# codex-storage/nim-groth16

Measured on AMD Instinct MI355X. Metric: proofs/sec (BN254 Groth16, 2^20-constraint circuit), higher is better.
Workload: dtype u32 (254-bit Montgomery: 8x32-bit limbs; 9x29-bit limbs in the bucket accumulation); 1 GPU; BN254 2^20-constraint synthetic R1CS (squaring chain, m=2^20-2), full prove: buildABC + 6 NTT + 4 G1 MSM + 1 G2 MSM, snarkjs flavour, 1 proof/step/GPU (3 proofs in flight per GPU, one shared key); mode=replica, nvars=1048576, domain_log2=20

## Files before the change

### include/g16hip.h

```cpp
#ifndef G16HIP_H
#define G16HIP_H

#include <stddef.h>
#include <stdint.h>

#ifdef __cplusplus
extern "C" {
#endif

#define G16_OK 0
#define G16_EINVAL (-1)
#define G16_ENODEV (-2)
#define G16_EHIP (-3)
#define G16_ENOMEM (-4)
#define G16_ESELFTEST (-5)

typedef struct g16_ctx g16_ctx;
typedef struct g16_points g16_points;

#define G16_SCALARS_MONT 1u
#define G16_SCALARS_STD 0u
#define G16_SCALARS_DEVICE 2u
#define G16_OUT_PARTIAL 4u
#define G16_OUT_DEVICE 8u
// ... 98 lines not shown
  const void *pointsA1, *pointsB1;
  const void* pointsB2;
  const void* pointsC1;
  const void* pointsH1;
  const g16_coeff* coeffs;
  size_t ncoeffs;
  const void *alpha1, *beta1, *delta1;
  const void *beta2, *delta2;
  uint32_t shard_index, shard_count;
} g16_pkey_desc;
typedef struct {
  uint8_t pi_a[64];
  uint8_t pi_b[128];
  uint8_t pi_c[64];
} g16_proof;
int32_t g16_pkey_create(g16_ctx* ctx, const g16_pkey_desc* desc, g16_pkey** out);
int32_t g16_pkey_create_zkey(g16_ctx* ctx, const g16_pkey_desc* desc, const void* section4, size_t section4_bytes,
                             g16_pkey** out);
int32_t g16_pkey_create_lean(g16_ctx* ctx, const g16_pkey_desc* desc, uint32_t table_stride, g16_pkey** out);
int32_t g16_pkey_create_zkey_lean(g16_ctx* ctx, const g16_pkey_desc* desc, const void* section4, size_t section4_bytes,
                                  uint32_t table_stride, g16_pkey** out);
void g16_pkey_destroy(g16_pkey* key);
int32_t g16_pkey_inf_counts(const g16_pkey* key, size_t out[8]);
int32_t g16_prove(g16_ctx* ctx, const g16_pkey* key, const void* witness, uint32_t flags, const void* mask_r,
                  const void* mask_s, g16_proof* out);
#define G16_PARTIALS_BYTES 768
int32_t g16_prove_partials(g16_ctx* ctx, const g16_pkey* key, const void* witness, uint32_t flags, void* out_partials);
int32_t g16_prove_combine(g16_ctx* ctx, const g16_pkey* key, const void* partials, size_t count, uint32_t flags,
                          const void* mask_r, const void* mask_s, g16_proof* out);
int32_t g16_prove_partials_begin(g16_ctx* ctx, const g16_pkey* key, const void* witness, uint32_t flags,
                                 uint32_t task_mask, void* d_task_out);
int32_t g16_prove_partials_end(g16_ctx* ctx, const g16_pkey* key, const void* d_a1_slice, const void* d_b1_slice,
                               const void* d_c1_slice, uint32_t flags, void* out_partials);
int32_t g16_build_abc(g16_ctx* ctx, const g16_pkey* key, const void* witness, uint32_t flags, void* out_abc);
int32_t g16_pkey_abc_info(const g16_pkey* key, size_t out[11]);
int32_t g16_spmv_fr(g16_ctx* ctx, const uint32_t* row, const uint32_t* col, const void* val, size_t nnz, const void* x,
                    size_t ncols, size_t nrows, void* y);

typedef struct g16_group g16_group;
typedef struct g16_group_pkey g16_group_pkey;
int32_t g16_group_create(const int32_t* devices, int32_t ndev, g16_group** out);
void g16_group_destroy(g16_group* group);
int32_t g16_group_size(const g16_group* group);
const char* g16_group_last_error(const g16_group* group);
int32_t g16_group_pkey_create(g16_group* group, const g16_pkey_desc* desc, g16_group_pkey** out);
int32_t g16_group_pkey_create_lean(g16_group* group, const g16_pkey_desc* desc, uint32_t table_stride,
// ... 71 lines not shown
```

### nim_groth16_amd/_lib.py

```python
from __future__ import annotations

import ctypes
import json
import os
import weakref

_HERE = os.path.dirname(os.path.abspath(__file__))

G16_OK, G16_EINVAL, G16_ENODEV, G16_EHIP, G16_ENOMEM, G16_ESELFTEST, G16_EBUSY = 0, -1, -2, -3, -4, -5, -6
SCALARS_MONT, SCALARS_STD, SCALARS_DEVICE, OUT_PARTIAL, OUT_DEVICE, NO_HOST_SYNC = 1, 0, 2, 4, 8, 32
PARTIALS_BYTES = 768

SYMBOLS = [
    "g16_ctx_create", "g16_ctx_destroy", "g16_last_error", "g16_ctx_set_stream", "g16_ctx_synchronize",
    "g16_selftest", "g16_msm_g1", "g16_msm_g2", "g16_msm_g1_dev", "g16_msm_g2_dev",
    "g16_msm_g1_partial_dev", "g16_msm_g2_partial_dev", "g16_g1_sum_partials", "g16_g2_sum_partials",
    "g16_points_register_g1", "g16_points_register_g2", "g16_points_register_g1_dev",
    "g16_points_register_g2_dev", "g16_points_release", "g16_points_count", "g16_points_inf_count", "g16_points_info", "g16_msm_points",
    "g16_points_check_g1", "g16_points_check_g2", "g16_fixed_base_g1", "g16_fixed_base_g2", "g16_quotient", "g16_quotient_dev", "g16_pkey_create",
    "g16_pkey_create_zkey", "g16_pkey_destroy", "g16_pkey_inf_counts", "g16_prove", "g16_build_abc", "g16_pkey_abc_info", "g16_spmv_fr", "g16_prove_partials", "g16_prove_combine",
    "g16_prove_partials_begin", "g16_prove_partials_end",
    "g16_ntt_fr", "g16_ntt_fr_dev", "g16_profile_enable", "g16_profile_reset", "g16_profile_report", "g16_profile_clock",
    "g16_vkey_create", "g16_vkey_destroy", "g16_verify", "g16_verify_batch", "g16_pairing",
    "g16_ctx_cancel", "g16_group_create", "g16_group_destroy", "g16_group_size", "g16_group_last_error",
    "g16_group_pkey_create", "g16_group_pkey_destroy", "g16_group_prove",
    "g16_prover_create", "g16_prover_destroy", "g16_prover_last_error", "g16_prover_submit", "g16_prover_poll",
    "g16_prover_collect", "g16_host_alloc", "g16_host_free",
    "g16_points_register_g1_lean", "g16_points_register_g2_lean", "g16_points_register_g1_lean_dev",
    "g16_points_register_g2_lean_dev", "g16_points_table_bytes", "g16_points_plan", "g16_pkey_create_lean",
    "g16_pkey_create_zkey_lean", "g16_group_pkey_create_lean",
    "g16_setup_log2_domain", "g16_fake_setup", "g16_lagrange_fr", "g16_powers_fr",
    "g16_points_audit_g1", "g16_points_audit_g2", "g16_points_pairs_check", "g16_key_audit",
]
VERIFY_SUBGROUP = 16
GT_BYTES = 384


class PkeyDesc(ctypes.Structure):
    _fields_ = [("nvars", ctypes.c_uint32), ("npubs", ctypes.c_uint32), ("log2_domain", ctypes.c_uint32),
                ("flavour", ctypes.c_uint32),
                ("pointsA1", ctypes.c_void_p), ("pointsB1", ctypes.c_void_p), ("pointsB2", ctypes.c_void_p),
                ("pointsC1", ctypes.c_void_p), ("pointsH1", ctypes.c_void_p),
                ("coeffs", ctypes.c_void_p), ("ncoeffs", ctypes.c_size_t),
                ("alpha1", ctypes.c_void_p), ("beta1", ctypes.c_void_p), ("delta1", ctypes.c_void_p),
                ("beta2", ctypes.c_void_p), ("delta2", ctypes.c_void_p),
                ("shard_index", ctypes.c_uint32), ("shard_count", ctypes.c_uint32)]


class VkeyDesc(ctypes.Structure):
    _fields_ = [("npubs", ctypes.c_uint32), ("alpha1", ctypes.c_void_p), ("beta2", ctypes.c_void_p),
                ("gamma2", ctypes.c_void_p), ("delta2", ctypes.c_void_p), ("pointsIC", ctypes.c_void_p)]


class SetupDesc(ctypes.Structure):
    _fields_ = [("nvars", ctypes.c_uint32), ("npubs", ctypes.c_uint32), ("nconstraints", ctypes.c_uint32),
# ... 128 lines not shown
    for name in ("g16_msm_g1", "g16_msm_g2", "g16_msm_g1_dev", "g16_msm_g2_dev",
                 "g16_msm_g1_partial_dev", "g16_msm_g2_partial_dev"):
        getattr(lib, name).argtypes = [vp, vp, u32, vp, sz, vp]
    for name in ("g16_g1_sum_partials", "g16_g2_sum_partials"):
        getattr(lib, name).argtypes = [vp, vp, sz, vp]
    for name in ("g16_points_register_g1", "g16_points_register_g2", "g16_points_register_g1_dev",
                 "g16_points_register_g2_dev"):
        getattr(lib, name).argtypes = [vp, vp, sz, ctypes.POINTER(vp)]
    for name in ("g16_points_register_g1_lean", "g16_points_register_g2_lean", "g16_points_register_g1_lean_dev",
                 "g16_points_register_g2_lean_dev"):
        getattr(lib, name).argtypes = [vp, vp, sz, u32, ctypes.POINTER(vp)]
    lib.g16_points_table_bytes.argtypes = [vp, ctypes.POINTER(sz)]
    lib.g16_points_plan.argtypes = [ctypes.c_int, sz, u32, ctypes.POINTER(u32), ctypes.POINTER(u32), ctypes.POINTER(sz)]
    lib.g16_pkey_create_lean.argtypes = [vp, ctypes.POINTER(PkeyDesc), u32, ctypes.POINTER(vp)]
    lib.g16_pkey_create_zkey_lean.argtypes = [vp, ctypes.POINTER(PkeyDesc), vp, sz, u32, ctypes.POINTER(vp)]
    lib.g16_group_pkey_create_lean.argtypes = [vp, ctypes.POINTER(PkeyDesc), u32, ctypes.POINTER(vp)]
    lib.g16_points_release.argtypes = [vp]
    lib.g16_points_release.restype = None
    lib.g16_points_count.argtypes = [vp]
    lib.g16_points_count.restype = sz
    lib.g16_points_inf_count.argtypes = [vp]
    lib.g16_points_inf_count.restype = sz
    lib.g16_pkey_inf_counts.argtypes = [vp, ctypes.POINTER(sz)]
    lib.g16_points_info.argtypes = [vp, ctypes.POINTER(u32), ctypes.POINTER(u32)]
    lib.g16_msm_points.argtypes = [vp, vp, vp, u32, vp]
    lib.g16_points_check_g1.argtypes = [vp, vp, sz, ctypes.POINTER(sz)]
    lib.g16_points_check_g2.argtypes = [vp, vp, sz, ctypes.POINTER(sz)]
    lib.g16_fixed_base_g1.argtypes = [vp, vp, u32, sz, vp]
    lib.g16_fixed_base_g2.argtypes = [vp, vp, u32, sz, vp]
    lib.g16_quotient.argtypes = [vp, vp, vp, vp, u32, u32, vp]
    lib.g16_quotient_dev.argtypes = [vp, vp, vp, vp, u32, u32, vp]
    lib.g16_pkey_create.argtypes = [vp, ctypes.POINTER(PkeyDesc), ctypes.POINTER(vp)]
    lib.g16_pkey_create_zkey.argtypes = [vp, ctypes.POINTER(PkeyDesc), vp, sz, ctypes.POINTER(vp)]
    lib.g16_pkey_destroy.argtypes = [vp]
    lib.g16_pkey_destroy.restype = None
    lib.g16_prove.argtypes = [vp, vp, vp, u32, vp, vp, vp]
    lib.g16_build_abc.argtypes = [vp, vp, vp, u32, vp]
    lib.g16_pkey_abc_info.argtypes = [vp, ctypes.POINTER(sz)]
    lib.g16_spmv_fr.argtypes = [vp, vp, vp, vp, sz, vp, sz, sz, vp]
    lib.g16_prove_partials.argtypes = [vp, vp, vp, u32, vp]
    lib.g16_prove_combine.argtypes = [vp, vp, vp, sz, u32, vp, vp, vp]
    lib.g16_prove_partials_begin.argtypes = [vp, vp, vp, u32, u32, vp]
    lib.g16_prove_partials_end.argtypes = [vp, vp, vp, vp, vp, u32, vp]
    lib.g16_ntt_fr.argtypes = [vp, vp, vp, u32, i32]
    lib.g16_ntt_fr_dev.argtypes = [vp, vp, vp, u32, i32]
    lib.g16_vkey_create.argtypes = [vp, ctypes.POINTER(VkeyDesc), ctypes.POINTER(vp)]
# ... 360 lines not shown
        if out is not None:
            c._check(c._lib.g16_prove_partials_end(c._h, self._h, ptr(a1), ptr(b1), ptr(c1),
                                                   OUT_DEVICE | (NO_HOST_SYNC if nosync else 0), _buf(out)))
            return None
        buf = ctypes.create_string_buffer(PARTIALS_BYTES)
        c._check(c._lib.g16_prove_partials_end(c._h, self._h, ptr(a1), ptr(b1), ptr(c1), 0, buf))
        return buf.raw

    def prove_combine(self, partials, count: int, r: bytes = None, s: bytes = None, device: bool = False, ctx=None):
        c = ctx or self.ctx
        out = ctypes.create_string_buffer(256)
        c._check(c._lib.g16_prove_combine(c._h, self._h, _buf(partials), count, SCALARS_DEVICE if device else 0,
                                          _buf(r) if r else None, _buf(s) if s else None, out))
        raw = out.raw
        return raw[0:64], raw[64:192], raw[192:256]

    def inf_counts(self) -> dict:
        out = (ctypes.c_size_t * 8)()
        self.ctx._check(self.ctx._lib.g16_pkey_inf_counts(self._h, out))
        v = list(out)
        return {"A1": v[0], "B1": v[1], "B2": v[2], "C1": v[3], "H1": v[4], "B1_and_B2": v[5],
                "compact_A": bool(v[6]), "compact_B": bool(v[7])}

    def abc_info(self) -> dict:
        out = (ctypes.c_size_t * 11)()
        self.ctx._check(self.ctx._lib.g16_pkey_abc_info(self._h, out))
        v = list(out)
        names = ("L<=1", "L=2", "L<=4", "L<=8", "L<=16", "L<=32", "L<=64", "L<=128", "L>128")
        return {"ncoeffs": v[0], "dict_values": v[1], "rows_by_terms": dict(zip(names, v[2:]))}

    def build_abc(self, witness: bytes, mont: bool = True, ctx=None):
        c = ctx or self.ctx
        self._check_len(witness)
        n = 1 << self.log2n
        out = ctypes.create_string_buffer(3 * n * 32)
        c._check(c._lib.g16_build_abc(c._h, self._h, _buf(witness), SCALARS_MONT if mont else 0, out))
        raw = out.raw
        return raw[: 32 * n], raw[32 * n: 64 * n], raw[64 * n:]

    def _free(self):
        if self._h:
            self.ctx._lib.g16_pkey_destroy(self._h)
        self._h = None

    destroy = _free

# ... 271 lines not shown
```

### nim_groth16_amd/csrc/g16_env.hpp

```cpp
#pragma once

struct G16Env {
  int msm_window = 0;
  int table_window = 0;
  int msm_seg = 0;
  char msm_sort = 0;
  int g1_lanes[3] = {3, 2, 0};
  char stream_prio[7] = "lhllln";
  int red_slice_log2 = 0;
  int inf_compact_pct = 10;
  int r2_width = -1;
  int ntt_tile = 2048;
  int quotient_first = 1;
  int lanes_after_quotient = 0;
  int g1_batch = 0;
  int mtab = 2;
  int chain_ch = 1;
  int tail_quad = 1;
  int red_chunk = 0;
  int cu_split = 0;
  int heavy_grid = 0;
  int cz_on_the_fly = 1;
  int abc_dict = 1;
  int g2_first = -1;
};
```

### nim_groth16_amd/csrc/g16hip.hip

```cpp
#include "g16_internal.hpp"
#include "ec.cuh"

using namespace g16;

static G16Env read_env() {
  G16Env e;
  auto num = [](const char* name, int lo, int hi) {
    const char* v = getenv(name);
    if (!v) return 0;
    int x = atoi(v);
    return x >= lo && x <= hi ? x : 0;
  };
  e.msm_window = num("G16_MSM_WINDOW", 5, 22);
  e.table_window = num("G16_TABLE_WINDOW", 5, 22);
  e.msm_seg = num("G16_MSM_SEG", 8, 4096);
  e.red_slice_log2 = num("G16_RED_SLICE", 8, 11);
  e.cu_split = num("G16_CU_SPLIT", 1, 24);
  e.heavy_grid = num("G16_HEAVY_GRID", 1, 4096);
  if (const char* v = getenv("G16_INF_COMPACT")) e.inf_compact_pct = atoi(v) < 0 ? 0 : atoi(v) > 101 ? 101 : atoi(v);
  if (const char* v = getenv("G16_R2_WIDTH")) e.r2_width = v[0] == '0' ? 0 : v[0] == '2' ? 2 : 1;
  if (const char* v = getenv("G16_LANES_AFTER_QUOTIENT")) e.lanes_after_quotient = v[0] != '0';
  if (const char* v = getenv("G16_QUOTIENT_FIRST")) e.quotient_first = v[0] != '0';
  if (const char* v = getenv("G16_G1_BATCH")) e.g1_batch = v[0] != '0';
  if (const char* v = getenv("G16_CHAIN_CH")) e.chain_ch = v[0] != '0';
  if (const char* v = getenv("G16_ABC_DICT")) e.abc_dict = v[0] != '0';
  if (const char* v = getenv("G16_CZ_FLY")) e.cz_on_the_fly = v[0] != '0';
  if (const char* v = getenv("G16_RED_CHUNK")) e.red_chunk = atoi(v) == 2 || atoi(v) == 4 || atoi(v) == 8 || atoi(v) == 16 ? atoi(v) : 0;
  if (const char* v = getenv("G16_TAIL_QUAD")) e.tail_quad = v[0] != '0';
  if (const char* v = getenv("G16_G2_FIRST")) e.g2_first = v[0] == '2' ? 2 : v[0] != '0';
  if (const char* v = getenv("G16_MTAB")) e.mtab = v[0] == '1' ? 1 : 2;
  if (const char* v = getenv("G16_NTT_TILE")) e.ntt_tile = atoi(v) == 1024 ? 1024 : atoi(v) == 4096 ? 4096 : 2048;
  if (const char* v = getenv("G16_MSM_SORT")) e.msm_sort = v[0];
  if (const char* v = getenv("G16_G1_LANES"))
    if (strlen(v) == 3 && strspn(v, "023") == 3)
      for (int i = 0; i < 3; ++i) e.g1_lanes[i] = v[i] - '0';
  if (const char* v = getenv("G16_STREAM_PRIO"))
    if (strlen(v) >= 6 && strspn(v, "hnl") >= 6) memcpy(e.stream_prio, v, 6);
  return e;
}
const G16Env& g16_env() {
  static const G16Env env = read_env();
  return env;
}

static hipError_t ctx_stream_create(Stream& out, int prio_index, bool front) {
  hipStream_t st = nullptr;
  hipError_t e;
  if (g16_env().cu_split <= 0) {
    int lo = 0, hi = 0;
    (void)hipDeviceGetStreamPriorityRange(&lo, &hi);
    e = hipStreamCreateWithPriority(&st, hipStreamNonBlocking, stream_priority(g16_env(), prio_index, lo, hi));
  } else {
// ... 534 lines not shown
```

### nim_groth16_amd/csrc/msm.cuh

```cuda
#pragma once
#include "ec29.cuh"
#include "msm_params.hpp"

namespace g16 {

#ifndef G16_ACC_BLOCK
#define G16_ACC_BLOCK 256
#endif
constexpr int ACC_BLOCK = G16_ACC_BLOCK;
#ifndef G16_G2_WAVES
#define G16_G2_WAVES 2
#endif

#ifndef G16_TAIL_PRIO
#define G16_TAIL_PRIO 0
#endif
__device__ __forceinline__ void tail_prio() {
#if G16_TAIL_PRIO
  __builtin_amdgcn_s_setprio(G16_TAIL_PRIO);
#endif
}
#ifndef G16_G1_WAVES
#define G16_G1_WAVES 4
#endif
// ... 439 lines not shown
msm_accum(const MsmBatch<C> B, MsmParams P, unsigned long long* __restrict__ clk) {
  using E = Ec29<C>;
  const MsmJob<C>& J = B.job[blockIdx.y];
  const typename E::Tab* __restrict__ points = J.points;
  const uint32_t* __restrict__ entries = J.entries;
  const uint32_t* __restrict__ offset = J.offset;
  unsigned long long t0 = 0, r0 = 0;
  const bool stamp = clk != nullptr && threadIdx.x == 0;
  if (stamp) t0 = __builtin_amdgcn_s_memtime(), r0 = __builtin_amdgcn_s_memrealtime();
  const uint32_t t = blockIdx.x * ACC_BLOCK + threadIdx.x;
  const uint32_t nx = J.info[1] < P.max_extra ? J.info[1] : P.max_extra;
  uint32_t b, s, slot;
  if (t < nx) {
    uint2 d = J.xseg[t];
    b = d.x;
    s = d.y;
    slot = P.nbuckets + t;
  } else {
    if (t - nx >= P.nbuckets) return;
    b = J.perm[t - nx];
    s = 0;
    slot = b;
  }
  uint32_t beg = offset[b], end = offset[b + 1];
  beg += s * P.seg;
  if (end > beg + P.seg) end = beg + P.seg;
  typename E::Acc acc = E::acc_inf();
  if (J.init != nullptr && s == 0) acc = J.init[b];
  for (uint32_t j = beg; j < end; ++j) {
    const uint32_t e = entries[j];
    E::madd(acc, points + (e & 0x7fffffffu), e >> 31);
  }
  J.partial[slot] = acc;
  if (stamp) {
    atomicAdd(&clk[0], __builtin_amdgcn_s_memtime() - t0);
    atomicAdd(&clk[1], __builtin_amdgcn_s_memrealtime() - r0);
  }
}

template <class C>
__global__ void __launch_bounds__(MSM_BLOCK) points_to29(const typename C::Aff* __restrict__ points, uint32_t n,
                                                         typename Ec29<C>::Tab* __restrict__ out) {
  uint32_t i = blockIdx.x * MSM_BLOCK + threadIdx.x;
  if (i < n) out[i] = Ec29<C>::tab_from_std(points[i]);
}

// ... 549 lines not shown
```

### nim_groth16_amd/csrc/msm_sort.hip

```cpp
#include "g16_internal.hpp"
#include "msm.cuh"

using namespace g16;

static_assert(MSM_FLAG_SCALARS_MONT == G16_SCALARS_MONT, "msm_plan.hpp and the C ABI disagree on the Montgomery flag");

int32_t g16_msm_sort(g16_ctx* ctx, hipStream_t st, const void* d_scalars, uint32_t flags, size_t n, uint32_t table_cfg,
                     g16_ctx::MsmSort& S, const uint32_t* d_live) {
  const G16Env& env = g16_env();
  const MsmParams P = msm_params(n, flags, table_cfg, env);
  const MsmSortPlan L = msm_sort_plan(P, env);
  S.P = P;
  Carver measure{nullptr}, bind{nullptr};
  msm_sort_layout(S, P, L, measure);
  if (int32_t rc = ensure(ctx, S.buf, measure.bytes)) return rc;
  bind.base = (char*)S.buf.p();
  msm_sort_layout(S, P, L, bind);
  const auto* scalars = (const u256*)d_scalars;
  if (!L.use_part) HIPCHK(ctx, hipMemsetAsync(S.count, 0, (char*)S.offset - (char*)S.count, st));
  HIPCHK(ctx, hipMemsetAsync(S.info, 0, 64, st));
  HIPCHK(ctx, hipMemsetAsync(S.ghist, 0, PERM_BINS * 4, st));
  const bool lean = P.tstride >= 2;
  if (L.use_part) {
    if (lean)
// ... 75 lines not shown
    msm_job_layout(J, P, T.nchunks, asz, psz29, bind);
    J.points = (const typename Ec29<C>::Tab*)runs[j].d_points;
    J.entries = S.entries;
    J.offset = S.offset;
    J.xseg = S.xseg;
    J.info = S.info;
    J.perm = S.perm;
    J.heavy = S.heavy;
    J.xoff = S.xoff;
    J.init = (const typename Ec29<C>::Acc*)runs[j].init_partial;
    J.out_aff = (typename C::Aff*)runs[j].d_out_aff;
    J.out_acc = (typename C::Acc*)runs[j].d_out_acc;
  }
  int32_t rc;
  if ((rc = stage_accum<C>(ctx, st, P, B, n_accum))) return rc;
  if ((rc = stage_heavy<C>(ctx, st, P, T, B, n_accum))) return rc;
  if (after_heavy) HIPCHK(ctx, hipEventRecord(after_heavy, st));
  if (!n_tail) return G16_OK;
  if ((rc = stage_reduce1<C>(ctx, st, P, T, B, n_tail))) return rc;
  return stage_reduce2_fold<C>(ctx, st, P, T, B, n_tail);
}
int32_t g16_msm_batch(g16_ctx* ctx, hipStream_t stream, int group, const g16_msm_run* runs, int n_accum, int n_tail,
                      hipEvent_t after_heavy) {
  return group == 1 ? msm_batch<G1>(ctx, stream, runs, n_accum, n_tail, after_heavy)
                    : msm_batch<G2>(ctx, stream, runs, n_accum, n_tail, after_heavy);
}

template <class C>
int32_t msm_device(g16_ctx* ctx, const void* d_scalars, uint32_t flags, const void* d_points, size_t n, void* d_out_aff,
                   void* d_out_acc, uint32_t table_c, const uint32_t* d_live) {
  ctx->sort[0].narrow_tail = false;
  int32_t rc = g16_msm_sort(ctx, ctx->stream, d_scalars, flags, n, table_c, ctx->sort[0], d_live);
  if (rc) return rc;
  if ((table_c & 0xffu) == 0 && n) {
    static_assert(sizeof(typename Ec29<C>::Tab) == sizeof(typename C::Aff), "packed entries: 64 / 128 B");
    if ((rc = ensure(ctx, ctx->stage_p29, n * sizeof(typename Ec29<C>::Tab)))) return rc;
    if ((rc = to29_device<C>(ctx, ctx->stream, d_points, n, ctx->stage_p29.p()))) return rc;
    d_points = ctx->stage_p29.p();
  }
  const g16_msm_run run{&ctx->sort[0], &ctx->lane[0].acc, d_points, d_out_aff, d_out_acc, nullptr};
  return msm_batch<C>(ctx, ctx->stream, &run, 1, 1, nullptr);
}
template int32_t msm_device<G1>(g16_ctx*, const void*, uint32_t, const void*, size_t, void*, void*, uint32_t, const uint32_t*);
template int32_t msm_device<G2>(g16_ctx*, const void*, uint32_t, const void*, size_t, void*, void*, uint32_t, const uint32_t*);
```

### nim_groth16_amd/csrc/proof_plan.hpp

```cpp
#pragma once
#include <stddef.h>
#include <stdint.h>

#include "g16_env.hpp"

namespace g16 {

inline bool points_sparse(size_t n_inf, size_t n, const G16Env& env) {
  return n_inf && n_inf * 100 >= (size_t)env.inf_compact_pct * n;
}
inline void stream_cu_mask(const G16Env& env, bool front, uint32_t mask[8]) {
  for (int w = 0; w < 8; ++w) mask[w] = 0;
  for (int bit = 0; bit < 256; ++bit)
    if ((bit / 8 < env.cu_split) == front) mask[bit / 32] |= 1u << (bit % 32);
}
inline int stream_priority(const G16Env& env, int index, int lo, int hi) {
  switch (env.stream_prio[index]) {
    case 'h': return hi;
    case 'l': return lo;
    default: return (lo + hi) / 2;
  }
}

constexpr int8_t PS_MAIN = 5;
enum ProofEvent : int8_t { EV_NONE = -1, EV_A, EV_B, EV_Q, EV_B2, EV_C, EV_G2, EV_COUNT, EV_DONE0 = EV_COUNT };
enum ProofRun : int8_t { RUN_A1, RUN_B1, RUN_C1, RUN_B2, RUN_H, RUN_COUNT };
enum ProofSort : int8_t { SORT_W = 0, SORT_H = 1, SORT_WA = 2, SORT_WB = 3 };

enum ProofOp : uint8_t {
  OP_UPLOAD,
  OP_WAIT,
  OP_RECORD,
  OP_SORT_W,
  OP_SORT_H,
  OP_BUILD_ABC,
  OP_QUOTIENT,
  OP_COSET,
  OP_POINTWISE,
  OP_MSM,
  OP_COPY_OUT,
  OP_HOST_SYNC,
};
struct ProofStep {
  uint8_t op;
  int8_t stream;
  int8_t a, b, c, d, e;
};

enum ProofEntry : int { PROOF_WHOLE, PROOF_BEGIN, PROOF_END };
struct ProofShape {
  size_t nw, nh;
  uint32_t log2n;
  bool liveA, liveB;
  bool cfg_equal;
};

constexpr size_t G2_FIRST_MAX = size_t(1) << 18;

constexpr int PROOF_PLAN_CAP = 48;
struct ProofPlan {
  int count = 0, cap = PROOF_PLAN_CAP;
  bool overflow = false;
  bool narrow_tail = true;
  int8_t sort_a = SORT_W, sort_b = SORT_W;
  ProofStep steps[PROOF_PLAN_CAP];

  void push(ProofOp op, int stream, int a = 0, int b = 0, int c = 0, int d = 0, int e = 0) {
    if (count >= cap || count >= PROOF_PLAN_CAP) {
      overflow = true;
      return;
    }
    steps[count++] = ProofStep{(uint8_t)op, (int8_t)stream, (int8_t)a, (int8_t)b, (int8_t)c, (int8_t)d, (int8_t)e};
  }
  void record(int stream, int ev) { push(OP_RECORD, stream, ev); }
  void wait(int stream, int ev) {
    for (int i = count - 1; i >= 0; --i) {
      const ProofStep& s = steps[i];
      if ((s.op == OP_RECORD && s.a == ev) || (s.op == OP_MSM && s.d == ev)) break;
      if (s.op == OP_WAIT && s.stream == stream && s.a == ev) return;
    }
    push(OP_WAIT, stream, ev);
  }
  void msm(int stream, int first, int n_accum, int n_tail, int after_heavy = EV_NONE, bool continues_c1 = false) {
    push(OP_MSM, stream, first, n_accum, n_tail, after_heavy, continues_c1);
  }
};

// ... 47 lines not shown
      p.record(PS_MAIN, EV_Q);
      p.wait(hs, EV_Q);
    }
    const bool chain = proof_chains_c_into_h(env, s);
    if (chain) p.wait(hs, EV_C);
    p.msm(hs, RUN_H, 1, 1, EV_NONE, chain);
    if (hs != PS_MAIN) {
      p.record(hs, EV_DONE0 + 4);
      p.wait(PS_MAIN, EV_DONE0 + 4);
    }
  }
  if (s.nw)
    for (int i = 0; i < proof_witness_lanes(env); ++i) p.wait(PS_MAIN, EV_DONE0 + i);
  p.push(OP_COPY_OUT, PS_MAIN);
  if (host_sync) p.push(OP_HOST_SYNC, PS_MAIN);
}

inline bool proof_plan_build(ProofPlan& p, const G16Env& env, ProofEntry entry, uint32_t task_mask, bool host_sync,
                             const ProofShape& s, int cap = PROOF_PLAN_CAP) {
  p = ProofPlan();
  p.cap = cap;
  p.sort_a = s.liveA ? SORT_WA : SORT_W;
  p.sort_b = s.liveB ? SORT_WB : SORT_W;
  if (entry == PROOF_END) {
    p.push(OP_POINTWISE, PS_MAIN);
    proof_plan_h_and_collect(p, env, s, false, host_sync);
    return !p.overflow;
  }
  p.push(OP_UPLOAD, PS_MAIN);
  p.record(PS_MAIN, EV_A);
  if (entry == PROOF_BEGIN) {
    if (task_mask) p.push(OP_BUILD_ABC, PS_MAIN, (task_mask & 4u) != 0);
    for (int v = 0; v < 3; ++v)
      if (task_mask & (1u << v)) p.push(OP_COSET, PS_MAIN, v);
    int after = EV_NONE;
    if (task_mask && env.quotient_first && env.lanes_after_quotient) p.record(PS_MAIN, after = EV_Q);
    proof_plan_witness(p, env, s, after);
    if (host_sync) p.push(OP_HOST_SYNC, PS_MAIN);
    return !p.overflow;
  }
  const int fly = s.log2n >= 1 && env.cz_on_the_fly ? 1 : 0;
  if (!env.quotient_first) proof_plan_witness(p, env, s, EV_NONE);
  p.push(OP_BUILD_ABC, PS_MAIN, fly == 0);
  p.push(OP_QUOTIENT, PS_MAIN, fly);
  if (env.quotient_first) {
    if (s.nh) p.push(OP_SORT_H, PS_MAIN);
// ... 10 lines not shown
```

### nim_groth16_amd/csrc/prover.hip

```cpp
#include <algorithm>
#include <cstddef>
#include <new>

#include "g16_internal.hpp"
#include "host_curve.hpp"

using namespace g16;

struct g16_pkey {
  int device = 0;
  uint32_t nvars = 0, npubs = 0, log2n = 0, flavour = 1;
  uint32_t shard_index = 0, shard_count = 1;
  size_t w_lo = 0, w_hi = 0;
  size_t h_lo = 0, h_hi = 0;
  g16_points *A1 = nullptr, *B1 = nullptr, *B2 = nullptr, *C1 = nullptr, *H1 = nullptr;
  g16_spmat* abc = nullptr;
  size_t ncoeffs = 0;
  g1_aff alpha1, beta1, delta1;
  g2_aff beta2, delta2;
  const uint32_t* liveA = nullptr;
  DevMem<uint32_t> liveB;
  size_t deadB = 0;
};

extern "C" void g16_pkey_destroy(g16_pkey* k) {
  if (!k) return;
  for (g16_points* p : {k->A1, k->B1, k->B2, k->C1, k->H1}) g16_points_release(p);
  (void)hipSetDevice(k->device);
  (void)hipDeviceSynchronize();
  g16_spmat_destroy(k->abc);
  delete k;
}

void g16_pkey_shape(const g16_pkey* k, int* device, uint32_t* nvars, uint32_t* shard_count) {
  *device = k->device;
  *nvars = k->nvars;
  *shard_count = k->shard_count;
}

extern "C" int32_t g16_pkey_inf_counts(const g16_pkey* k, size_t out[8]) {
  if (!k || !out) return G16_EINVAL;
  const size_t pub_end = std::min<size_t>(k->w_hi, (size_t)k->npubs + 1);
  const size_t pad = pub_end > k->w_lo ? pub_end - k->w_lo : 0;
  out[0] = k->A1->n_inf, out[1] = k->B1->n_inf, out[2] = k->B2->n_inf, out[3] = k->C1->n_inf - pad, out[4] = k->H1->n_inf;
  out[5] = k->deadB, out[6] = k->liveA ? 1 : 0, out[7] = k->liveB ? 1 : 0;
  return G16_OK;
}

extern "C" int32_t g16_pkey_abc_info(const g16_pkey* k, size_t out[11]) {
  if (!k || !out) return G16_EINVAL;
  out[0] = k->ncoeffs;
  g16_spmat_info(k->abc, out + 1);
  return G16_OK;
}

struct CoeffSource {
  const unsigned char* base = nullptr;
  size_t count = 0, stride = 0, value_off = 0;
  bool values_r2 = false;
};
static inline uint32_t rd32(const unsigned char* p) {
  uint32_t v;
  memcpy(&v, p, 4);
  return v;
}

static int32_t pkey_create(g16_ctx* ctx, const g16_pkey_desc* d, const CoeffSource& cs, uint32_t table_stride,
                           g16_pkey** out) {
  const size_t n = size_t(1) << d->log2_domain;
  if (d->log2_domain > 27 || d->nvars == 0 || d->npubs + 1 > d->nvars || d->flavour > 1 || !d->pointsA1 ||
      !d->pointsB1 || !d->pointsB2 || !d->pointsH1 || (d->nvars - d->npubs - 1 > 0 && !d->pointsC1) ||
      !d->alpha1 || !d->beta1 || !d->delta1 || !d->beta2 || !d->delta2) {
    ctx->err = "bad proving-key description";
    return G16_EINVAL;
  }
  CTX_ENTER(ctx);
  Building<g16_pkey, g16_pkey_destroy> k(new (std::nothrow) g16_pkey());
  if (!k) return G16_ENOMEM;
  k->device = ctx->device;
  k->nvars = d->nvars;
  k->npubs = d->npubs;
  k->log2n = d->log2_domain;
  k->flavour = d->flavour;
  memcpy(&k->alpha1, d->alpha1, 64);
  memcpy(&k->beta1, d->beta1, 64);
  memcpy(&k->delta1, d->delta1, 64);
  memcpy(&k->beta2, d->beta2, 128);
  memcpy(&k->delta2, d->delta2, 128);
  int32_t rc;
  k->shard_count = d->shard_count ? d->shard_count : 1;
  k->shard_index = d->shard_index;
  if (k->shard_index >= k->shard_count) {
    ctx->err = "shard_index >= shard_count";
    return G16_EINVAL;
  }
  auto range = [&](size_t N, size_t& lo, size_t& hi) {
    lo = (N * k->shard_index) / k->shard_count;
    hi = (N * (k->shard_index + 1)) / k->shard_count;
  };
  range(d->nvars, k->w_lo, k->w_hi);
  range(n, k->h_lo, k->h_hi);
  std::vector<unsigned char> c1pad((k->w_hi - k->w_lo) * 64, 0);
  for (size_t wI = k->w_lo; wI < k->w_hi; ++wI)
    if (wI > d->npubs) memcpy(&c1pad[(wI - k->w_lo) * 64], (const char*)d->pointsC1 + 64 * (wI - d->npubs - 1), 64);
  const uint32_t ts = table_stride;
  if ((rc = g16_points_register_g1_lean(ctx, (const char*)d->pointsA1 + 64 * k->w_lo, k->w_hi - k->w_lo, ts, &k->A1))) return rc;
  if ((rc = g16_points_register_g1_lean(ctx, (const char*)d->pointsB1 + 64 * k->w_lo, k->w_hi - k->w_lo, ts, &k->B1))) return rc;
  if ((rc = g16_points_register_g2_lean(ctx, (const char*)d->pointsB2 + 128 * k->w_lo, k->w_hi - k->w_lo, ts, &k->B2))) return rc;
  if ((rc = g16_points_register_g1_lean(ctx, c1pad.data(), k->w_hi - k->w_lo, ts, &k->C1))) return rc;
  if ((rc = g16_points_register_g1_lean(ctx, (const char*)d->pointsH1 + 64 * k->h_lo, k->h_hi - k->h_lo, ts, &k->H1))) return rc;
  {
    const size_t nw = k->w_hi - k->w_lo;
    k->liveA = g16_points_live_if_sparse(k->A1);
    if (nw && k->B1->d_live && k->B2->d_live) {
      uint32_t dead = 0;
      if ((rc = ensure(ctx, ctx->stage_o, 2048))) return rc;
      uint32_t* d_cnt = (uint32_t*)ctx->stage_o.p();
      HIPCHK(ctx, dev_alloc(k->liveB, ((nw + 31) / 32 + 1) * 4));
      HIPCHK(ctx, hipMemsetAsync(d_cnt, 0, 4, ctx->stream));
      if ((rc = g16_bitmap_or_device(ctx, k->liveB.get(), k->B1->d_live.get(), k->B2->d_live.get(), nw, d_cnt))) return rc;
      HIPCHK(ctx, hipMemcpyAsync(&dead, d_cnt, 4, hipMemcpyDeviceToHost, ctx->stream));
      HIPCHK(ctx, hipStreamSynchronize(ctx->stream));
      k->deadB = dead;
      if (!points_sparse(dead, nw, g16_env())) k->liveB.reset();
    }
  }
  std::vector<uint32_t> vrow;
  try {
    vrow.resize(cs.count ? cs.count : 1);
  } catch (const std::bad_alloc&) {
    ctx->err = "out of host memory";
    return G16_ENOMEM;
  }
  for (size_t e = 0; e < cs.count; ++e) {
    const unsigned char* ent = cs.base + e * cs.stride;
    const uint32_t matrix = rd32(ent), row = rd32(ent + 4), col = rd32(ent + 8);
    if (matrix > 1 || row >= n || col >= d->nvars) {
// ... 57 lines not shown
extern "C" int32_t g16_build_abc(g16_ctx* ctx, const g16_pkey* k, const void* witness, uint32_t flags, void* out_abc) {
  if (!ctx) return G16_EINVAL;
  if (!k || !witness || !out_abc || k->device != ctx->device) {
    ctx->err = "bad argument";
    return G16_EINVAL;
  }
  CTX_ENTER(ctx);
  const size_t n = size_t(1) << k->log2n;
  int32_t rc;
  if ((rc = ensure(ctx, ctx->prove, ((size_t)k->nvars + 4 * n) * 32))) return rc;
  u256* d_w = (u256*)ctx->prove.p();
  u256* d_abc = d_w + k->nvars;
  HIPCHK(ctx, hipMemcpyAsync(d_w, witness, (size_t)k->nvars * 32, hipMemcpyHostToDevice, ctx->stream));
  if ((rc = build_abc_device(ctx, k, d_w, (flags & G16_SCALARS_MONT) ? 1u : 0u, d_abc))) return rc;
  HIPCHK(ctx, hipMemcpyAsync(out_abc, d_abc, 3 * n * 32, hipMemcpyDeviceToHost, ctx->stream));
  HIPCHK(ctx, hipStreamSynchronize(ctx->stream));
  return G16_OK;
}

static constexpr size_t PART_A = 0, PART_B1 = 128, PART_B2 = 256, PART_H = 512, PART_C = 640, PART_BYTES = 768;

static ProofShape proof_shape(const g16_pkey* k) {
  return ProofShape{k->w_hi - k->w_lo, k->h_hi - k->h_lo, k->log2n, k->liveA != nullptr, (bool)k->liveB,
                    k->C1->cfg() == k->H1->cfg()};
}

struct ProofArgs {
  const void* witness = nullptr;
  uint32_t flags = 0;
  u256* task_out = nullptr;
  const void *d_a1 = nullptr, *d_b1 = nullptr, *d_c1 = nullptr;
  bool qs_is_slice = false;
  void* out_partials = nullptr;
};

static int32_t run_plan(g16_ctx* ctx, const g16_pkey* k, ProofEntry entry, uint32_t task_mask, bool host_sync,
                        const ProofArgs& a) {
  ProofPlan plan;
  if (!proof_plan_build(plan, g16_env(), entry, task_mask, host_sync, proof_shape(k))) {
    ctx->err = "proof launch plan exceeds its capacity";
    return G16_EINVAL;
  }
  const size_t n = size_t(1) << k->log2n, nw = k->w_hi - k->w_lo, nh = k->h_hi - k->h_lo;
  int32_t rc;
  if ((rc = ensure(ctx, ctx->prove, ((size_t)k->nvars + 4 * n) * 32))) return rc;
  if ((rc = ensure(ctx, ctx->stage_o, 2048))) return rc;
  u256* const d_w = (u256*)ctx->prove.p();
  u256* const d_abc = d_w + k->nvars;
  u256* const d_qs = d_abc + 3 * n;
  char* const slots = (char*)ctx->stage_o.p();
  const u256* const d_wr = d_w + k->w_lo;
  const u256* const d_qs_slice = a.qs_is_slice ? d_qs : d_qs + k->h_lo;
  const uint32_t wit_mont = (a.flags & G16_SCALARS_MONT) ? 1u : 0u;
  g16_ctx::MsmLane* L = ctx->lane;
  const g16_points* const sets[RUN_COUNT] = {k->A1, k->B1, k->C1, k->B2, k->H1};
  g16_msm_run runs[RUN_COUNT] = {
      {&ctx->sort[plan.sort_a], &L[0].acc, k->A1->d_tables.get(), nullptr, slots + PART_A, nullptr},
      {&ctx->sort[plan.sort_b], &L[2].acc, k->B1->d_tables.get(), nullptr, slots + PART_B1, nullptr},
      {&ctx->sort[SORT_W], &L[3].acc, k->C1->d_tables.get(), nullptr, slots + PART_C, nullptr},
      {&ctx->sort[plan.sort_b], &L[1].acc, k->B2->d_tables.get(), nullptr, slots + PART_B2, nullptr},
      {&ctx->sort[SORT_H], &L[4].acc, k->H1->d_tables.get(), nullptr, slots + PART_H, nullptr}};
  auto event = [&](int e) { return e == EV_NONE ? nullptr : e < EV_COUNT ? ctx->ev[e].get() : L[e - EV_DONE0].done.get(); };
  for (int i = 0; i < plan.count; ++i) {
    const ProofStep& s = plan.steps[i];
    rc = G16_OK;
    hipStream_t st = s.stream == PS_MAIN ? ctx->stream : L[s.stream].stream.get();
    switch (s.op) {
      case OP_UPLOAD:
        HIPCHK(ctx, hipMemcpyAsync(d_w, a.witness, (size_t)k->nvars * 32,
                                   (a.flags & G16_SCALARS_DEVICE) ? hipMemcpyDeviceToDevice : hipMemcpyHostToDevice, st));
        HIPCHK(ctx, hipMemsetAsync(slots, 0, PART_BYTES, st));
        break;
      case OP_WAIT: HIPCHK(ctx, hipStreamWaitEvent(st, event(s.a), 0)); break;
      case OP_RECORD: HIPCHK(ctx, hipEventRecord(event(s.a), st)); break;
      case OP_SORT_W:
        ctx->sort[s.a].narrow_tail = plan.narrow_tail;
        rc = g16_msm_sort(ctx, st, d_wr, wit_mont ? G16_SCALARS_MONT : 0u, nw, sets[s.c]->cfg(), ctx->sort[s.a],
                          s.b == 0 ? nullptr : s.b == 1 ? k->liveA : k->liveB.get());
        break;
      case OP_SORT_H:
        ctx->sort[SORT_H].narrow_tail = plan.narrow_tail;
// ... 65 lines not shown
}

extern "C" int32_t g16_prove_partials_end(g16_ctx* ctx, const g16_pkey* k, const void* d_a1, const void* d_b1,
                                          const void* d_c1, uint32_t flags, void* out_partials) {
  if (!ctx) return G16_EINVAL;
  const size_t nh = k ? k->h_hi - k->h_lo : 0;
  if (!k || !out_partials || k->device != ctx->device || (nh && (!d_a1 || !d_b1 || !d_c1))) {
    ctx->err = "bad argument";
    return G16_EINVAL;
  }
  if (ctx->shard_begun != k) {
    ctx->err = "g16_prove_partials_end without a matching g16_prove_partials_begin on this context";
    return G16_EINVAL;
  }
  CTX_ENTER_KEEP(ctx);
  ctx->shard_begun = nullptr;
  ProofArgs a;
  a.flags = flags, a.d_a1 = d_a1, a.d_b1 = d_b1, a.d_c1 = d_c1, a.qs_is_slice = true, a.out_partials = out_partials;
  const int32_t rc = run_plan(ctx, k, PROOF_END, 0, !((flags & G16_NO_HOST_SYNC) && (flags & G16_OUT_DEVICE)), a);
  if (rc != G16_OK) ctx_quiesce(ctx);
  return rc;
}

static __global__ void prove_combine_kernel(const unsigned char* __restrict__ gathered, uint32_t count,
                                            unsigned char* __restrict__ out) {
  if (threadIdx.x != 0) return;
  const uint32_t b = blockIdx.x;
  if (b == 2) {
    g2_acc r = G2::acc_inf();
    for (uint32_t i = 0; i < count; ++i) G2::add(r, *(const g2_acc*)(gathered + (size_t)i * PART_BYTES + PART_B2));
    *(g2_aff*)(out + 128) = G2::to_affine(r);
  } else {
    const size_t src = b == 0 ? PART_A : b == 1 ? PART_B1 : b == 3 ? PART_H : PART_C;
    const size_t dst = b == 0 ? 0 : b == 1 ? 64 : b == 3 ? 256 : 320;
    g1_acc r = G1::acc_inf();
    for (uint32_t i = 0; i < count; ++i) G1::add(r, *(const g1_acc*)(gathered + (size_t)i * PART_BYTES + src));
    *(g1_aff*)(out + dst) = G1::to_affine(r);
  }
}

static_assert(sizeof(CombineRes) == G16_COMBINE_RES_BYTES, "slot layout");
static_assert(sizeof(CombinePre) == sizeof(g16_combine_pre), "g16_combine_pre layout");

int32_t g16_combine_enqueue(g16_ctx* ctx, const g16_pkey* k, const void* partials, size_t count, uint32_t flags,
                            const void* mask_r, const void* mask_s, void* res_host, hipEvent_t done,
                            g16_combine_pre* pre_out) {
  int32_t rc;
  if ((rc = ensure(ctx, ctx->stage_p, count * PART_BYTES))) return rc;
  if ((rc = ensure(ctx, ctx->stage_o, 2048))) return rc;
  HIPCHK(ctx, hipMemcpyAsync(ctx->stage_p.p(), partials, count * PART_BYTES,
                             (flags & G16_SCALARS_DEVICE) ? hipMemcpyDeviceToDevice : hipMemcpyHostToDevice,
                             ctx->stream));
  unsigned char* d_res = (unsigned char*)ctx->stage_o.p() + 1024;
  KLAUNCH(ctx, "prove_combine", prove_combine_kernel, 5, 64, 0, (const unsigned char*)ctx->stage_p.p(), (uint32_t)count,
          d_res);

  u256 r = Fr::zero(), s = Fr::zero();
  if (mask_r) memcpy(&r, mask_r, 32);
  if (mask_s) memcpy(&s, mask_s, 32);
  const CombinePre pre = host_combine_pre(k->alpha1, k->beta1, k->delta1, k->beta2, k->delta2, r, s);
  memcpy(pre_out, &pre, sizeof pre);
  HIPCHK(ctx, hipMemcpyAsync(res_host, d_res, sizeof(CombineRes), hipMemcpyDeviceToHost, ctx->stream));
  if (done) HIPCHK(ctx, hipEventRecord(done, ctx->stream));
  return G16_OK;
}

void g16_combine_finish(const g16_combine_pre* pre_in, const void* res_host, g16_proof* out) {
  CombinePre pre;
  CombineRes res;
  memcpy(&pre, pre_in, sizeof pre);
  memcpy(&res, res_host, sizeof res);
  g1_aff pi_a, pi_c;
  g2_aff pi_b;
  host_combine_finish(pre, res, pi_a, pi_b, pi_c);
  memcpy(out->pi_a, &pi_a, 64);
  memcpy(out->pi_b, &pi_b, 128);
  memcpy(out->pi_c, &pi_c, 64);
}
// ... 71 lines not shown
```

Baseline: 118.0 proofs/s.

## Fold B1 query into A1 via point differences and skip empty B1 MSM

```diff
diff --git a/include/g16hip.h b/include/g16hip.h
--- a/include/g16hip.h
+++ b/include/g16hip.h
@@ -144,6 +144,7 @@
                                   uint32_t table_stride, g16_pkey** out);
 void g16_pkey_destroy(g16_pkey* key);
 int32_t g16_pkey_inf_counts(const g16_pkey* key, size_t out[8]);
+int32_t g16_pkey_b1_fold(const g16_pkey* key, size_t out[3]);
 int32_t g16_prove(g16_ctx* ctx, const g16_pkey* key, const void* witness, uint32_t flags, const void* mask_r,
                   const void* mask_s, g16_proof* out);
 #define G16_PARTIALS_BYTES 768
diff --git a/nim_groth16_amd/_lib.py b/nim_groth16_amd/_lib.py
--- a/nim_groth16_amd/_lib.py
+++ b/nim_groth16_amd/_lib.py
@@ -31,6 +31,7 @@
     "g16_pkey_create_zkey_lean", "g16_group_pkey_create_lean",
     "g16_setup_log2_domain", "g16_fake_setup", "g16_lagrange_fr", "g16_powers_fr",
     "g16_points_audit_g1", "g16_points_audit_g2", "g16_points_pairs_check", "g16_key_audit",
+    "g16_pkey_b1_fold",
 ]
 VERIFY_SUBGROUP = 16
 GT_BYTES = 384
@@ -205,6 +206,7 @@
     lib.g16_points_inf_count.argtypes = [vp]
     lib.g16_points_inf_count.restype = sz
     lib.g16_pkey_inf_counts.argtypes = [vp, ctypes.POINTER(sz)]
+    lib.g16_pkey_b1_fold.argtypes = [vp, ctypes.POINTER(sz)]
     lib.g16_points_info.argtypes = [vp, ctypes.POINTER(u32), ctypes.POINTER(u32)]
     lib.g16_msm_points.argtypes = [vp, vp, vp, u32, vp]
     lib.g16_points_check_g1.argtypes = [vp, vp, sz, ctypes.POINTER(sz)]
@@ -611,6 +613,11 @@
         return {"A1": v[0], "B1": v[1], "B2": v[2], "C1": v[3], "H1": v[4], "B1_and_B2": v[5],
                 "compact_A": bool(v[6]), "compact_B": bool(v[7])}
 
+    def b1_fold(self) -> dict:
+        out = (ctypes.c_size_t * 3)()
+        self.ctx._check(self.ctx._lib.g16_pkey_b1_fold(self._h, out))
+        return {"form": ("PLAIN", "EMPTY", "DELTA")[out[0]], "live_b1": out[1], "live_delta": out[2]}
+
     def abc_info(self) -> dict:
         out = (ctypes.c_size_t * 11)()
         self.ctx._check(self.ctx._lib.g16_pkey_abc_info(self._h, out))
diff --git a/nim_groth16_amd/csrc/b1_fold.cuh b/nim_groth16_amd/csrc/b1_fold.cuh
--- /dev/null
+++ b/nim_groth16_amd/csrc/b1_fold.cuh
@@ -0,0 +1,17 @@
+#pragma once
+#include "ec.cuh"
+
+namespace g16 {
+
+template <class C>
+FF_HD typename C::Aff point_difference(const typename C::Aff& b, const typename C::Aff& a) {
+  using F = typename C::Field;
+  if (F::eq(a.x, b.x) && F::eq(a.y, b.y)) return C::aff_inf();
+  if (C::is_inf(a)) return b;
+  if (C::is_inf(b)) return C::neg(a);
+  typename C::Acc acc = C::from_affine(b);
+  C::madd(acc, C::neg(a));
+  return C::to_affine(acc);
+}
+
+}
diff --git a/nim_groth16_amd/csrc/g16_env.hpp b/nim_groth16_amd/csrc/g16_env.hpp
--- a/nim_groth16_amd/csrc/g16_env.hpp
+++ b/nim_groth16_amd/csrc/g16_env.hpp
@@ -23,4 +23,5 @@
   int cz_on_the_fly = 1;
   int abc_dict = 1;
   int g2_first = -1;
+  int b1_fold = 1;
 };
diff --git a/nim_groth16_amd/csrc/g16hip.hip b/nim_groth16_amd/csrc/g16hip.hip
--- a/nim_groth16_amd/csrc/g16hip.hip
+++ b/nim_groth16_amd/csrc/g16hip.hip
@@ -28,6 +28,7 @@
   if (const char* v = getenv("G16_RED_CHUNK")) e.red_chunk = atoi(v) == 2 || atoi(v) == 4 || atoi(v) == 8 || atoi(v) == 16 ? atoi(v) : 0;
   if (const char* v = getenv("G16_TAIL_QUAD")) e.tail_quad = v[0] != '0';
   if (const char* v = getenv("G16_G2_FIRST")) e.g2_first = v[0] == '2' ? 2 : v[0] != '0';
+  if (const char* v = getenv("G16_B1_FOLD")) e.b1_fold = v[0] != '0';
   if (const char* v = getenv("G16_MTAB")) e.mtab = v[0] == '1' ? 1 : 2;
   if (const char* v = getenv("G16_NTT_TILE")) e.ntt_tile = atoi(v) == 1024 ? 1024 : atoi(v) == 4096 ? 4096 : 2048;
   if (const char* v = getenv("G16_MSM_SORT")) e.msm_sort = v[0];
diff --git a/nim_groth16_amd/csrc/msm.cuh b/nim_groth16_amd/csrc/msm.cuh
--- a/nim_groth16_amd/csrc/msm.cuh
+++ b/nim_groth16_amd/csrc/msm.cuh
@@ -485,6 +485,10 @@
     s = 0;
     slot = b;
   }
+  if (points == nullptr) {
+    J.partial[slot] = E::acc_inf();
+    return;
+  }
   uint32_t beg = offset[b], end = offset[b + 1];
   beg += s * P.seg;
   if (end > beg + P.seg) end = beg + P.seg;
diff --git a/nim_groth16_amd/csrc/msm_sort.hip b/nim_groth16_amd/csrc/msm_sort.hip
--- a/nim_groth16_amd/csrc/msm_sort.hip
+++ b/nim_groth16_amd/csrc/msm_sort.hip
@@ -121,6 +121,11 @@
 }
 int32_t g16_msm_batch(g16_ctx* ctx, hipStream_t stream, int group, const g16_msm_run* runs, int n_accum, int n_tail,
                       hipEvent_t after_heavy) {
+  for (int i = 0; i < n_accum; ++i)
+    if (!runs[i].d_points && runs[i].init_partial) {
+      ctx->err = "an MSM run without a table cannot continue another run's bucket sums";
+      return G16_EINVAL;
+    }
   return group == 1 ? msm_batch<G1>(ctx, stream, runs, n_accum, n_tail, after_heavy)
                     : msm_batch<G2>(ctx, stream, runs, n_accum, n_tail, after_heavy);
 }
diff --git a/nim_groth16_amd/csrc/proof_plan.hpp b/nim_groth16_amd/csrc/proof_plan.hpp
--- a/nim_groth16_amd/csrc/proof_plan.hpp
+++ b/nim_groth16_amd/csrc/proof_plan.hpp
@@ -8,6 +8,16 @@
 
 inline bool points_sparse(size_t n_inf, size_t n, const G16Env& env) {
   return n_inf && n_inf * 100 >= (size_t)env.inf_compact_pct * n;
+}
+enum B1Form : int { B1_PLAIN = 0, B1_EMPTY = 1, B1_DELTA = 2 };
+inline B1Form b1_fold_form(size_t live_b1, size_t live_delta, size_t n, const G16Env& env) {
+  if (!env.b1_fold) return B1_PLAIN;
+  if (live_delta == 0) return B1_EMPTY;
+  const long long keep = 100 - (long long)env.inf_compact_pct;
+  if ((long long)live_delta * 100 > (long long)live_b1 * keep) return B1_PLAIN;
+  const bool b1_compacted = n >= live_b1 && points_sparse(n - live_b1, n, env);
+  if (b1_compacted && live_delta * 64 > live_b1) return B1_PLAIN;
+  return B1_DELTA;
 }
 inline void stream_cu_mask(const G16Env& env, bool front, uint32_t mask[8]) {
   for (int w = 0; w < 8; ++w) mask[w] = 0;
@@ -53,6 +63,7 @@
   uint32_t log2n;
   bool liveA, liveB;
   bool cfg_equal;
+  int b1_form = B1_PLAIN;
 };
 
 constexpr size_t G2_FIRST_MAX = size_t(1) << 18;
@@ -63,6 +74,7 @@
   bool overflow = false;
   bool narrow_tail = true;
   int8_t sort_a = SORT_W, sort_b = SORT_W;
+  int8_t sort_b1 = SORT_W;
   ProofStep steps[PROOF_PLAN_CAP];
 
   void push(ProofOp op, int stream, int a = 0, int b = 0, int c = 0, int d = 0, int e = 0) {
@@ -156,6 +168,7 @@
   p.cap = cap;
   p.sort_a = s.liveA ? SORT_WA : SORT_W;
   p.sort_b = s.liveB ? SORT_WB : SORT_W;
+  p.sort_b1 = s.b1_form == B1_PLAIN ? p.sort_b : SORT_W;
   if (entry == PROOF_END) {
     p.push(OP_POINTWISE, PS_MAIN);
     proof_plan_h_and_collect(p, env, s, false, host_sync);
diff --git a/nim_groth16_amd/csrc/prover.hip b/nim_groth16_amd/csrc/prover.hip
--- a/nim_groth16_amd/csrc/prover.hip
+++ b/nim_groth16_amd/csrc/prover.hip
@@ -3,6 +3,7 @@
 #include <new>
 
 #include "g16_internal.hpp"
+#include "b1_fold.cuh"
 #include "host_curve.hpp"
 
 using namespace g16;
@@ -21,6 +22,9 @@
   const uint32_t* liveA = nullptr;
   DevMem<uint32_t> liveB;
   size_t deadB = 0;
+  int b1_form = B1_PLAIN;
+  size_t b1_inf = 0;
+  size_t live_b1 = 0, live_delta = 0;
 };
 
 extern "C" void g16_pkey_destroy(g16_pkey* k) {
@@ -42,8 +46,14 @@
   if (!k || !out) return G16_EINVAL;
   const size_t pub_end = std::min<size_t>(k->w_hi, (size_t)k->npubs + 1);
   const size_t pad = pub_end > k->w_lo ? pub_end - k->w_lo : 0;
-  out[0] = k->A1->n_inf, out[1] = k->B1->n_inf, out[2] = k->B2->n_inf, out[3] = k->C1->n_inf - pad, out[4] = k->H1->n_inf;
+  out[0] = k->A1->n_inf, out[1] = k->b1_inf, out[2] = k->B2->n_inf, out[3] = k->C1->n_inf - pad, out[4] = k->H1->n_inf;
   out[5] = k->deadB, out[6] = k->liveA ? 1 : 0, out[7] = k->liveB ? 1 : 0;
+  return G16_OK;
+}
+
+extern "C" int32_t g16_pkey_b1_fold(const g16_pkey* k, size_t out[3]) {
+  if (!k || !out) return G16_EINVAL;
+  out[0] = (size_t)k->b1_form, out[1] = k->live_b1, out[2] = k->live_delta;
   return G16_OK;
 }
 
@@ -63,6 +73,33 @@
   uint32_t v;
   memcpy(&v, p, 4);
   return v;
+}
+
+static __global__ void __launch_bounds__(256) b1_compare_kernel(const uint4* __restrict__ a1, const uint4* __restrict__ b1,
+                                                                uint32_t n, uint32_t* __restrict__ cnt) {
+  const uint32_t i = blockIdx.x * 256 + threadIdx.x;
+  bool live = false, differs = false;
+  if (i < n) {
+    uint32_t any = 0, diff = 0;
+#pragma unroll
+    for (int q = 0; q < 4; ++q) {
+      const uint4 a = a1[(size_t)i * 4 + q], b = b1[(size_t)i * 4 + q];
+      any |= b.x | b.y | b.z | b.w;
+      diff |= (a.x ^ b.x) | (a.y ^ b.y) | (a.z ^ b.z) | (a.w ^ b.w);
+    }
+    live = any != 0, differs = diff != 0;
+  }
+  const uint32_t nl = (uint32_t)__popcll(__ballot(live)), nd = (uint32_t)__popcll(__ballot(differs));
+  if ((threadIdx.x & 63) == 0) {
+    if (nl) atomicAdd(&cnt[0], nl);
+    if (nd) atomicAdd(&cnt[1], nd);
+  }
+}
+static __global__ void __launch_bounds__(256) b1_delta_kernel(const g1_aff* __restrict__ a1, g1_aff* __restrict__ b1,
+                                                              uint32_t n) {
+  const uint32_t i = blockIdx.x * 256 + threadIdx.x;
+  if (i >= n) return;
+  b1[i] = point_difference<G1>(b1[i], a1[i]);
 }
 
 static int32_t pkey_create(g16_ctx* ctx, const g16_pkey_desc* d, const CoeffSource& cs, uint32_t table_stride,
@@ -105,14 +142,73 @@
     if (wI > d->npubs) memcpy(&c1pad[(wI - k->w_lo) * 64], (const char*)d->pointsC1 + 64 * (wI - d->npubs - 1), 64);
   const uint32_t ts = table_stride;
   if ((rc = g16_points_register_g1_lean(ctx, (const char*)d->pointsA1 + 64 * k->w_lo, k->w_hi - k->w_lo, ts, &k->A1))) return rc;
-  if ((rc = g16_points_register_g1_lean(ctx, (const char*)d->pointsB1 + 64 * k->w_lo, k->w_hi - k->w_lo, ts, &k->B1))) return rc;
+  {
+    const size_t nv = d->nvars, nw = k->w_hi - k->w_lo;
+    SyncOnExit sync{ctx->stream};
+    uint32_t cnt[2] = {0, 0};
+    if (g16_env().b1_fold) {
+      constexpr size_t CHUNK = size_t(1) << 16;
+      const size_t step = std::min(nv, CHUNK);
+      DevMem<g1_aff> c_a1, c_b1;
+      SyncOnExit sync_chunks{ctx->stream};
+      if ((rc = ensure(ctx, ctx->stage_o, 2048))) return rc;
+      uint32_t* d_cnt = (uint32_t*)ctx->stage_o.p();
+      HIPCHK(ctx, dev_alloc(c_a1, step * sizeof(g1_aff)));
+      HIPCHK(ctx, dev_alloc(c_b1, step * sizeof(g1_aff)));
+      HIPCHK(ctx, hipMemsetAsync(d_cnt, 0, 8, ctx->stream));
+      for (size_t lo = 0; lo < nv; lo += step) {
+        const size_t m = std::min(step, nv - lo);
+        HIPCHK(ctx, hipMemcpyAsync(c_a1.get(), (const char*)d->pointsA1 + 64 * lo, m * 64, hipMemcpyHostToDevice, ctx->stream));
+        HIPCHK(ctx, hipMemcpyAsync(c_b1.get(), (const char*)d->pointsB1 + 64 * lo, m * 64, hipMemcpyHostToDevice, ctx->stream));
+        hipLaunchKernelGGL(b1_compare_kernel, dim3((uint32_t)((m + 255) / 256)), dim3(256), 0, ctx->stream,
+                           (const uint4*)c_a1.get(), (const uint4*)c_b1.get(), (uint32_t)m, d_cnt);
+        HIPCHK(ctx, hipGetLastError());
+      }
+      HIPCHK(ctx, hipMemcpyAsync(cnt, d_cnt, 8, hipMemcpyDeviceToHost, ctx->stream));
+      HIPCHK(ctx, hipStreamSynchronize(ctx->stream));
+    }
+    k->live_b1 = cnt[0], k->live_delta = cnt[1];
+    k->b1_form = b1_fold_form(cnt[0], cnt[1], nv, g16_env());
+    if (k->b1_form == B1_DELTA && nw) {
+      DevMem<g1_aff> d_a1, d_b1;
+      SyncOnExit sync_arrays{ctx->stream};
+      HIPCHK(ctx, dev_alloc(d_a1, nw * sizeof(g1_aff)));
+      HIPCHK(ctx, dev_alloc(d_b1, nw * sizeof(g1_aff)));
+      HIPCHK(ctx, hipMemcpyAsync(d_a1.get(), (const char*)d->pointsA1 + 64 * k->w_lo, nw * 64, hipMemcpyHostToDevice, ctx->stream));
+      HIPCHK(ctx, hipMemcpyAsync(d_b1.get(), (const char*)d->pointsB1 + 64 * k->w_lo, nw * 64, hipMemcpyHostToDevice, ctx->stream));
+      uint32_t n_inf = 0;
+      DevMem<uint32_t> scratch_live;
+      uint32_t* d_cnt = (uint32_t*)ctx->stage_o.p();
+      HIPCHK(ctx, dev_alloc(scratch_live, ((nw + 31) / 32 + 1) * 4));
+      HIPCHK(ctx, hipMemsetAsync(d_cnt, 0, 4, ctx->stream));
+      if ((rc = live_bitmap_device<G1>(ctx, d_b1.get(), nw, scratch_live.get(), d_cnt))) return rc;
+      HIPCHK(ctx, hipMemcpyAsync(&n_inf, d_cnt, 4, hipMemcpyDeviceToHost, ctx->stream));
+      hipLaunchKernelGGL(b1_delta_kernel, dim3((uint32_t)((nw + 255) / 256)), dim3(256), 0, ctx->stream,
+                         (const g1_aff*)d_a1.get(), d_b1.get(), (uint32_t)nw);
+      HIPCHK(ctx, hipGetLastError());
+      HIPCHK(ctx, hipStreamSynchronize(ctx->stream));
+      k->b1_inf = n_inf;
+      if ((rc = g16_points_register_g1_lean_dev(ctx, d_b1.get(), nw, ts, &k->B1))) return rc;
+    } else {
+      if ((rc = g16_points_register_g1_lean(ctx, (const char*)d->pointsB1 + 64 * k->w_lo, nw, ts, &k->B1))) return rc;
+      k->b1_inf = k->B1->n_inf;
+    }
+  }
   if ((rc = g16_points_register_g2_lean(ctx, (const char*)d->pointsB2 + 128 * k->w_lo, k->w_hi - k->w_lo, ts, &k->B2))) return rc;
   if ((rc = g16_points_register_g1_lean(ctx, c1pad.data(), k->w_hi - k->w_lo, ts, &k->C1))) return rc;
   if ((rc = g16_points_register_g1_lean(ctx, (const char*)d->pointsH1 + 64 * k->h_lo, k->h_hi - k->h_lo, ts, &k->H1))) return rc;
   {
     const size_t nw = k->w_hi - k->w_lo;
     k->liveA = g16_points_live_if_sparse(k->A1);
-    if (nw && k->B1->d_live && k->B2->d_live) {
+    if (nw && k->b1_form == B1_DELTA && k->B2->d_live) {
+      k->deadB = k->B2->n_inf;
+      if (points_sparse(k->deadB, nw, g16_env())) {
+        const size_t words = (nw + 31) / 32 + 1;
+        HIPCHK(ctx, dev_alloc(k->liveB, words * 4));
+        HIPCHK(ctx, hipMemcpyAsync(k->liveB.get(), k->B2->d_live.get(), words * 4, hipMemcpyDeviceToDevice, ctx->stream));
+        HIPCHK(ctx, hipStreamSynchronize(ctx->stream));
+      }
+    } else if (nw && k->B1->d_live && k->B2->d_live) {
       uint32_t dead = 0;
       if ((rc = ensure(ctx, ctx->stage_o, 2048))) return rc;
       uint32_t* d_cnt = (uint32_t*)ctx->stage_o.p();
@@ -216,7 +312,7 @@
 
 static ProofShape proof_shape(const g16_pkey* k) {
   return ProofShape{k->w_hi - k->w_lo, k->h_hi - k->h_lo, k->log2n, k->liveA != nullptr, (bool)k->liveB,
-                    k->C1->cfg() == k->H1->cfg()};
+                    k->C1->cfg() == k->H1->cfg(), k->b1_form};
 }
 
 struct ProofArgs {
@@ -250,7 +346,8 @@
   const g16_points* const sets[RUN_COUNT] = {k->A1, k->B1, k->C1, k->B2, k->H1};
   g16_msm_run runs[RUN_COUNT] = {
       {&ctx->sort[plan.sort_a], &L[0].acc, k->A1->d_tables.get(), nullptr, slots + PART_A, nullptr},
-      {&ctx->sort[plan.sort_b], &L[2].acc, k->B1->d_tables.get(), nullptr, slots + PART_B1, nullptr},
+      {&ctx->sort[plan.sort_b1], &L[2].acc, k->b1_form == B1_EMPTY ? nullptr : k->B1->d_tables.get(), nullptr,
+       slots + PART_B1, nullptr},
       {&ctx->sort[SORT_W], &L[3].acc, k->C1->d_tables.get(), nullptr, slots + PART_C, nullptr},
       {&ctx->sort[plan.sort_b], &L[1].acc, k->B2->d_tables.get(), nullptr, slots + PART_B2, nullptr},
       {&ctx->sort[SORT_H], &L[4].acc, k->H1->d_tables.get(), nullptr, slots + PART_H, nullptr}};
@@ -362,7 +459,7 @@
   return rc;
 }
 
-static __global__ void prove_combine_kernel(const unsigned char* __restrict__ gathered, uint32_t count,
+static __global__ void prove_combine_kernel(const unsigned char* __restrict__ gathered, uint32_t count, uint32_t fold_b1,
                                             unsigned char* __restrict__ out) {
   if (threadIdx.x != 0) return;
   const uint32_t b = blockIdx.x;
@@ -375,6 +472,8 @@
     const size_t dst = b == 0 ? 0 : b == 1 ? 64 : b == 3 ? 256 : 320;
     g1_acc r = G1::acc_inf();
     for (uint32_t i = 0; i < count; ++i) G1::add(r, *(const g1_acc*)(gathered + (size_t)i * PART_BYTES + src));
+    if (b == 1 && fold_b1)
+      for (uint32_t i = 0; i < count; ++i) G1::add(r, *(const g1_acc*)(gathered + (size_t)i * PART_BYTES + PART_A));
     *(g1_aff*)(out + dst) = G1::to_affine(r);
   }
 }
@@ -393,7 +492,7 @@
                              ctx->stream));
   unsigned char* d_res = (unsigned char*)ctx->stage_o.p() + 1024;
   KLAUNCH(ctx, "prove_combine", prove_combine_kernel, 5, 64, 0, (const unsigned char*)ctx->stage_p.p(), (uint32_t)count,
-          d_res);
+          k->b1_form != B1_PLAIN ? 1u : 0u, d_res);
 
   u256 r = Fr::zero(), s = Fr::zero();
   if (mask_r) memcpy(&r, mask_r, 32);
```

Measured after the change: 129.0 proofs/s, median of 6. 9.3% higher.
